# MobleyLab/blues

Measured on AMD Instinct MI355X. Metric: NCMC ns/day (23k-atom toluene box, 1000-step switch, RandomLigandRotationMove), aggregate over independent chains, higher is better.
Workload: dtype f32 pair math / f64 accumulation, f64 alchemical+integrator

## Files before the change

blues_amd/csrc/blues_engine.hip:

```cpp
#include <hip/hip_runtime.h>

#include <algorithm>
#include <array>
#include <cmath>
#include <cstdarg>
#include <cstdio>
#include <cstdlib>
#include <cstring>
#include <map>
#include <memory>
#include <numeric>
#include <string>
#include <vector>

#include "../../include/blues_engine.h"
#include "device_common.h"
#include "kernels_alch.h"
#include "kernels_bonded.h"
#include <chrono>
#include <mutex>
#include <thread>
#include <functional>
#include <atomic>
#include <type_traits>
// ... 234 lines not shown
    bool clusters_packed = false;
    double total_mass = 0;
    DBuf<double> d_x[3], d_v[3], d_xbuild[3], d_mass, d_charge, d_sigma, d_eps;
    DBuf<double> d_x_sort[3], d_stage;
    DBuf<unsigned> d_xfer_out;
    DBuf<int> d_edit_idx; DBuf<double> d_edit_xyz;
    std::vector<struct BluesSnapshot*> snap_pool;
    DBuf<AtomF> d_img_f; DBuf<AtomD> d_img_d;
    DBuf<int> d_sorted_of_orig, d_orig_of_sorted, d_tile_atoms, d_jlist, d_jstage, d_jcount, d_batch_slot, d_ex_start, d_ex_idx, d_islot;
    DBuf<unsigned long long> d_mask_pool;
    DBuf<DevFlags> d_flags; DBuf<DevAccum> d_acc; DBuf<long long> d_stamps;
    DBuf<double> d_fpart, d_epart_nb, d_fJ, d_self_part, d_e_part, d_fent, d_ftot, d_alch_self, d_epart_b, d_cm_part, d_trace, d_scratch;
    DBuf<int> d_orig_of_islot, d_row_of_orig, d_mobile_atoms, d_mobile_index, d_exc_owner, d_exc_is_env;
    DBuf<double> d_noise; unsigned noise_draw_base = 0; int n_noise = 0; bool noise_valid = false;
    DBuf<int> d_alch_orig, d_alch_local, d_exc_start, d_exc_partner; DBuf<double> d_exc_params;
    DBuf<int> d_cl_atoms, d_cl_type, d_cl_nc, d_cl_alch, d_cl_mobile, d_cl_sorted; DBuf<double> d_cl_dist;
    DBuf<ClusterRec> d_recs; std::vector<ClusterRec> h_recs;
    std::vector<GenCluster> gen_h; std::vector<GenAtom> gen_atoms_h; std::vector<GenCons> gen_cons_h;
    std::vector<int> gen_tree;
    DBuf<GenCluster> d_gen; DBuf<GenAtom> d_gen_atoms; DBuf<GenCons> d_gen_cons;
    int n_gen() const { return (int)gen_h.size(); }
    int gen_blocks() const { const int wpb = int_threads / 64; return (n_gen() + wpb - 1) / wpb; }
    DBuf<AlchJRec> d_jrec; DBuf<AlchARec> d_arec;
    DBuf<double> d_mom_part; bool vel_clean = false, pass_valid_for_l = true;
    DBuf<FinRec> d_finrecs; std::vector<int> h_row_of_orig, h_row_start;
    template <typename T> struct PmeBufs { DBuf<T> a_re, a_im, b_re, b_im, eterm, tw_cos[3], tw_sin[3], qf_re, qf_im, phi_f; };
    bool pme = false; int pme_K[3] = {0, 0, 0}, pme_order = 5, disp_corr = 0;
    std::vector<int> pme_frozen;
    DBuf<double> d_qn, d_qn_full, d_frec, d_pme_e; DBuf<int> d_pme_frozen; DBuf<unsigned long long> d_pme_acc;
    PmeBufs<float> pme_f; PmeBufs<double> pme_d;
    bool pme_static_valid = false;
    double e_ewald_const = 0.0, e_disp = 0.0;
    DBuf<int> d_row_atom, d_row_start, d_ent_type, d_ent_term, d_ent_role;
    DBuf<int> d_term_atoms[T_NTYPES]; DBuf<double> d_term_params[T_NTYPES];
    int n_terms[T_NTYPES] = {0, 0, 0, 0, 0, 0}; int n_rows = 0; double restr_k = 0;
    int n_cent = 0; DBuf<int> d_cent_atoms; DBuf<double> d_cent_params;
    Program prog; unsigned prog_draw_base = 0; int prog_trace = -1; bool tracing = false;
    int64_t st_passes = 0, st_launches = 0, st_resorts = 0, st_energy_evals = 0, st_reshapes = 0;
    std::vector<int> h_sorted_of_orig, h_orig_of_sorted;

    ~BluesEngine() {
        for (BluesSnapshot* sn : snap_pool) { if (sn->block) hipFree(sn->block); delete sn; }
        for (hipEvent_t e : {ev0, ev1, evFork, evJ1, evJ2, evA, evB}) if (e) hipEventDestroy(e);
        for (hipStream_t q : {s1, s2}) if (q) hipStreamDestroy(q);
    }
};
// ... 774 lines not shown
            A.q = (float)q; A.hs = (float)hs; A.se = (float)se; A.flags = flags; A.orig = o;
        } else {
            AtomD& A = imd[s];
            A.x = u[0]; A.y = u[1]; A.z = u[2]; A.q = q; A.hs = hs; A.se = se; A.flags = flags; A.orig = o; A.pad = 0;
        }
    }
    try {
        if (h->precision == 0) h->d_img_f.upload(imf); else h->d_img_d.upload(imd);
        h->d_sorted_of_orig.upload(h->h_sorted_of_orig); h->d_orig_of_sorted.upload(h->h_orig_of_sorted);
        { std::vector<int> cs(h->clusters.size() * 4, 0);
          for (size_t c = 0; c < h->clusters.size(); c++) for (int a = 0; a < 4; a++) if (h->clusters[c].atoms[a] >= 0) cs[c * 4 + a] = h->h_sorted_of_orig[h->clusters[c].atoms[a]];
          h->d_cl_sorted.upload(cs);
          for (size_t c = 0; c < h->clusters.size(); c++) for (int a = 0; a < 4; a++) {
              const int at = h->clusters[c].atoms[a];
              h->h_recs[c].sorted[a] = cs[c * 4 + a]; h->h_recs[c].islot[a] = at >= 0 ? islot[at] : -1;
              const int row = at >= 0 && !h->h_row_of_orig.empty() ? h->h_row_of_orig[at] : -1;
              h->h_recs[c].e0[a] = row >= 0 ? h->h_row_start[row] : 0; h->h_recs[c].e1[a] = row >= 0 ? h->h_row_start[row + 1] : 0;
          }
          h->d_recs.upload(h->h_recs); }
        if (h->n_gen()) { for (GenAtom& R : h->gen_atoms_h) { R.sorted = h->h_sorted_of_orig[R.atom]; R.islot = islot[R.atom]; } h->d_gen_atoms.upload(h->gen_atoms_h); }
        h->d_tile_atoms.upload(tile_atoms); h->d_islot.upload(islot);
        h->d_ex_start.upload(ex_start); h->d_ex_idx.upload(ex_idx);
        h->d_jrec.alloc((size_t)jcap);
        { std::vector<AlchARec> ar(h->alch.size());
          for (size_t a2 = 0; a2 < h->alch.size(); a2++) { AlchARec& r = ar[a2]; const int ao = h->alch[a2]; r.ao = ao; r.asrt = h->h_sorted_of_orig[ao]; r.pad = 0; r.sig = h->T->sigma[ao]; r.eps = std::sqrt(h->T->eps[ao]); r.q = h->T->charge[ao];
            r.has_env_excl = 0; for (int p2 : h->T->excl[ao]) if (h->T->alch_local[p2] < 0) r.has_env_excl = 1; }
          h->d_arec.upload(ar); }
        h->lists_alloc = h->k1_mode == 2 ? std::max(1, h->n_itiles) : 0;
        const int nt_alloc = h->k1_mode == 2 ? h->lists_alloc + 1 : nt;
        h->d_jlist.alloc((size_t)nt_alloc * jcap); h->d_jstage.alloc((size_t)nt_alloc * LIST_WAVES * ((((n + LIST_WAVES - 1) / LIST_WAVES) + 63) & ~63)); h->d_jcount.alloc(nt_alloc); h->d_batch_slot.alloc((size_t)nt_alloc * (jcap / 64));
        h->d_mask_pool.alloc((size_t)nt_alloc * MASK_QUOTA * 64);
        h->d_fpart.alloc((size_t)h->npart * 3 * h->n_islots);
        if (h->k1_mode == 2) {
            h->d_alist.alloc((size_t)h->n_islots * h->acap); h->d_acount.alloc(h->n_islots); h->d_aself.alloc(h->n_islots);
            {
                std::vector<int> rows((size_t)h->n_islots * SX_ROW, -1);
                for (int q = 0; q < h->n_islots; q++) {
                    int* r = rows.data() + (size_t)q * SX_ROW;
                    const int sidx = tile_atoms[q];
                    r[28] = 0; r[29] = 0x7fffffff; r[30] = -1;
                    if (sidx < 0) continue;
                    int nrow = 0; r[nrow++] = sidx;
                    for (int e = ex_start[sidx]; e < ex_start[sidx + 1]; e++) if (ex_idx[e] != sidx && nrow < SX_MAX) r[nrow++] = ex_idx[e];
                    r[28] = nrow;
                    for (int e = 0; e < nrow; e++) { r[29] = std::min(r[29], r[e]); r[30] = std::max(r[30], r[e]); }
                }
// ... 188 lines not shown
    h->prog.n = 0; h->prog_trace = -1; h->prog_draw_base = h->h_draw;
    HIP_OK(h, hipGetLastError());
    return 0;
}

static int emit(BluesEngine* h, int op) {
    if (h->prog.n == 0) h->prog_draw_base = h->h_draw;
    if (h->prog.n >= MAX_OPS) { if (flush_program(h)) return 1; h->prog_draw_base = h->h_draw; }
    h->prog.ops[h->prog.n++] = (unsigned char)op;
    if (op == OP_O || op == OP_L) h->h_draw++;
    return 0;
}

static ListArgs make_list_args(BluesEngine* h) {
    ListArgs a; memset(&a, 0, sizeof a);
    a.n = h->n; a.n_tiles = h->n_tiles; a.n_itiles = h->n_itiles; a.jcap = h->jcap; a.pool_cap = h->pool_cap;
    a.tile_atoms = h->d_tile_atoms.p; a.jlist = h->d_jlist.p; a.jstage = h->d_jstage.p; a.jcount = h->d_jcount.p; a.batch_slot = h->d_batch_slot.p;
    a.mask_pool = h->d_mask_pool.p; a.batch_req = batch_req_ptr(h); a.ex_start = h->d_ex_start.p; a.ex_idx = h->d_ex_idx.p; a.flags = h->d_flags.p;
    for (int k = 0; k < 3; k++) { a.x[k] = h->d_x[k].p; a.xbuild[k] = h->d_xbuild[k].p; }
    a.fJ = h->d_fJ.p; a.n_fJ = 9 * h->n;
    a.alch_jrec = h->alch.empty() ? nullptr : (void*)h->d_jrec.p; a.p_sigma = h->d_sigma.p; a.p_eps = h->d_eps.p; a.p_charge = h->d_charge.p;
    if (h->k1_mode == 2) { a.alist = h->d_alist.p; a.acount = h->d_acount.p; a.acap = h->acap; }
    a.S = h->S; a.n_lists = h->n_lists; a.hint_count = h->hint_count; a.no_sphere = h->tune.no_sphere;
    if (h->k1_mode == 2 && h->prune_on) { a.pneed = h->d_pneed.p; a.plist = h->d_plist.p; a.pcount = h->d_pcount.p; for (int k = 0; k < 3; k++) a.xprune[k] = h->d_xprune[k].p; }
    if (h->k1_mode == 2) { a.pimg4 = h->d_pimg4.p; a.pimg2 = h->d_pimg2.p; a.mlist = h->d_mlist.p; a.mcount = h->d_mcount.p; a.mcap = h->mcap; a.aself = h->d_aself.p; a.pimgb = h->d_pimgb.p; a.sx_row = h->d_sx_row.p; a.pf_reach = h->alist_pf_reach; }
    return a;
}

static FragArgs make_frag_args(BluesEngine* h) {
    FragArgs a; memset(&a, 0, sizeof a);
    if (h->k1_mode != 3) return a;
    a.F = h->frag_F; a.NI = h->frag_NI; a.ifrag = h->d_ifrag.p; a.nblk = h->frag_nblk; a.n = h->n; a.ocap = h->frag_ocap; a.icap = h->frag_icap; a.fpw = h->frag_fpw; a.nwg = h->frag_nwg; a.n_islots = h->n_islots;
    a.fimg = h->d_fimg.p; a.ljtab = h->d_ljtab.p; a.ntypes = h->frag_ntypes; a.sp_start = h->d_sp_start.p; a.sp_ent = h->d_sp_ent.p; a.bb = h->d_fbb.p; a.fpos0 = h->d_fpos0.p;
    a.olist = h->d_olist.p; a.ocount = h->d_ocount.p; a.ilist = h->d_ilist.p; a.icount = h->d_icount.p; a.xprune = h->d_xprune_s.p;
    const double ro = h->cutoff + h->skin, ri = h->cutoff + std::min(h->frag_m, h->skin);
    a.ro2 = (float)(ro * ro) * 1.0001f + 1e-5f; a.ri2 = (float)(ri * ri) * 1.0001f + 1e-5f;
    {
        const double rof = h->cutoff + 0.5 * h->skin, rif = h->cutoff + 0.5 * std::min(h->frag_m, h->skin);
        a.ro2_f = (float)(rof * rof) * 1.0001f + 1e-5f; a.ri2_f = (float)(rif * rif) * 1.0001f + 1e-5f;
    }
    a.ptrig2 = h->frag_m < h->skin ? (float)(0.25 * h->frag_m * h->frag_m) : 1e30f;
    for (int k = 0; k < 3; k++) a.scale[k] = (float)(h->box[k] / 4294967296.0);
    a.flags = h->d_flags.p; a.batch_req = batch_req_ptr(h); a.fpart = h->d_fpart.p; a.epart = h->d_epart_nb.p;
    a.half_min_edge = (float)(0.5 * std::min(h->box[0], std::min(h->box[1], h->box[2])));
    a.count_builds = h->n_tiles == 0;
    a.hint_blocks = h->frag_nblk < 64 ? 0x7fffffff : std::max(48, h->frag_nblk * 85 / 100);
// ... 307 lines not shown
        else hipLaunchKernelGGL(k_alchemical<false>, dim3(h->k2_nblocks_env + 1), dim3(256), 0, h->cur, A);
    }
    h->st_launches++;
    HIP_OK(h, hipGetLastError());
    return 0;
}

static AlchArgs make_alch_args(BluesEngine* h, const double ls[3], const double le[3], int slot_mask) {
    AlchArgs A; memset(&A, 0, sizeof A);
    A.jrec = h->d_jrec.p; A.arec = h->d_arec.p;
    A.n = h->n; A.n_alch = (int)h->alch.size(); A.PA = h->PA; A.jcap = h->jcap; A.nblocks_env = h->k2_nblocks_env; A.jiter = h->k2_jiter;
    A.flags_overflow = h->d_flags.p ? &h->d_flags.p->list_overflow : nullptr;
    A.alch_orig = h->d_alch_orig.p; A.jlist = h->d_jlist.p + (size_t)h->n_lists * h->jcap; A.jcount = h->d_jcount.p + h->n_lists;
    A.orig_of_sorted = h->d_orig_of_sorted.p; A.sorted_of_orig = h->d_sorted_of_orig.p;
    for (int k = 0; k < 3; k++) A.x[k] = h->d_x[k].p;
    A.charge = h->d_charge.p; A.sigma = h->d_sigma.p; A.eps = h->d_eps.p; A.ex_start = h->d_ex_start.p; A.ex_idx = h->d_ex_idx.p;
    A.exc_start = h->d_exc_start.p; A.exc_partner = h->d_exc_partner.p; A.exc_owner = h->d_exc_owner.p; A.exc_is_env = h->d_exc_is_env.p; A.exc_params = h->d_exc_params.p;
    A.box = make_box(h); A.rc2 = nocut(h) ? 1e300 : h->cutoff * h->cutoff; A.alpha = h->alpha; A.sc_alpha = h->sc_alpha;
    A.pme = h->nb_method == BLUES_NB_PME_DIRECT; A.annih_elec = h->annih_elec; A.annih_ster = h->annih_ster; A.slot_mask = slot_mask; A.check_env_excl = h->check_env_excl;
    for (int s = 0; s < 3; s++) { A.ls[s] = ls[s]; A.le[s] = le[s]; }
    A.fJ = h->d_fJ.p; A.self_part = h->d_self_part.p; A.e_part = h->d_e_part.p;
    A.img = h->precision == 0 ? h->d_img_f.p : nullptr;
    for (int k = 0; k < 3; k++) A.fscale[k] = (float)(h->box[k] / 4294967296.0);
    return A;
}

static BondedArgs make_bonded_args(BluesEngine* h) {
    BondedArgs B; memset(&B, 0, sizeof B);
    B.n_rows = h->n_rows; B.row_atom = h->d_row_atom.p; B.row_start = h->d_row_start.p;
    B.ent_type = h->d_ent_type.p; B.ent_term = h->d_ent_term.p; B.ent_role = h->d_ent_role.p;
    for (int ty = 0; ty < T_NTYPES; ty++) { B.n_terms[ty] = h->n_terms[ty]; B.atoms[ty] = h->d_term_atoms[ty].p; B.params[ty] = h->d_term_params[ty].p; }
    B.restr_k = h->restr_k; B.ewald_alpha = h->alpha;
    for (int k = 0; k < 3; k++) B.x[k] = h->d_x[k].p;
    B.box = make_box(h); B.periodic = h->nb_method == BLUES_NB_PME_DIRECT; B.fent = h->d_fent.p; B.n_entries = h->n_entries; B.n = h->n; B.epart = h->d_epart_b.p;
    B.n_mobile = (int)h->mobile.size(); B.n_noise = h->n_noise; B.mobile_atoms = h->d_mobile_atoms.p; B.noise = h->d_noise.p;
    B.n_cent = h->n_cent; B.cent_atoms = h->d_cent_atoms.p; B.cent_params = h->d_cent_params.p;
    B.seed = h->seed; B.stream = (unsigned)h->replica * 4u; B.draw_base = h->h_draw; B.n_entry_blocks = (h->n_entries + 127) / 128;
    return B;
}

static int launch_bonded(BluesEngine* h, bool with_noise) {
    BondedArgs B = make_bonded_args(h);
    const int nb_noise = with_noise ? ((int)h->mobile.size() * h->n_noise + 127) / 128 : 0;
    if (with_noise) { h->noise_draw_base = h->h_draw; h->noise_valid = true; }
    if (B.n_entry_blocks + nb_noise > 0) {
        BondedDyn D; D.draw_base = B.draw_base; D.n_entry_blocks = B.n_entry_blocks;
// ... 1876 lines not shown
    else if (k == "nprop") *value = h->nprop;
    else if (k == "prop") *value = h->h_prop;
    else if (k == "prop_lambda_min") *value = h->prop_min;
    else if (k == "prop_lambda_max") *value = h->prop_max;
    else if (k == "Enew" || k == "Eold") {
        double E; if (total_energy(h, &E)) return 1;
        if (read_acc(h, &a)) return 1;
        *value = (k == "Enew") ? E : E - a.dE_last;
    }
    else if (k == "heat") { if (h->led_flags & LED_HEAT) { if (read_acc(h, &a)) return 1; *value = a.heat; } else *value = 0.0; }
    else if (k == "kT") *value = h->kT;
    else if (h->switch_mode != BLUES_SWITCH_NONE && (k == "total_work" || k == "Epert" || k == "initial_energy" || k == "final_energy" || k == "accept" || k == "naccept" || k == "ntrials" || k == "psteps")) {
        if (k == "total_work") { if (read_acc(h, &a)) return 1; *value = a.protocol_work + h->sw_shadow; }
        else if (k == "Epert") *value = h->sw_Epert;
        else if (k == "initial_energy") *value = h->sw_Einit;
        else if (k == "final_energy") { if (h->h_step == 0) *value = 0.0; else if (h->psteps > 0) *value = h->sw_Epert; else if (total_energy(h, value)) return 1; }
        else if (k == "accept") *value = h->sw_accept;
        else if (k == "naccept") *value = h->sw_naccept;
        else if (k == "ntrials") *value = h->sw_ntrials;
        else *value = h->psteps;
    }
    else if (k == "lambda_sterics") *value = h->cur_ls;
    else if (k == "lambda_electrostatics") *value = h->cur_le;
    else E_FAIL(h, "unknown global variable '%s'", name);
    return 0;
}

int blues_set_global(BluesEngine* h, const char* name, double value) {
    HIP_OK(h, hipSetDevice(h->device));
    std::string k(name);
    if (k == "atom_list_prefilter") { h->alist_pf_reach = value <= 0.0 ? -1.0f : (float)(std::min(value, 1e5) * 1e-3); return 0; }
    if (k == "protocol_work" || (k == "shadow_work" && (h->led_flags & LED_SHADOW)) || (k == "heat" && (h->led_flags & LED_HEAT))) {
        DevAccum a; if (read_acc(h, &a)) return 1;
        if (k == "protocol_work") a.protocol_work = value; else if (k == "heat") a.heat = value; else a.shadow_work = value;
        HIP_OK(h, hipMemcpy(h->d_acc.p, &a, sizeof a, hipMemcpyHostToDevice));
        h->acc_cache_valid = false;
    }
    else if (k == "step") h->h_step = (int)value;
    else if (k == "lambda") h->h_lambda = value;
    else if (k == "lambda_step") { h->h_lambda_step = (int)value; parameters_changed(h); }
    else if (k == "first_step") h->h_first_step = (int)value;
    else if (k == "prop") h->h_prop = (int)value;
    else if (k == "nprop") h->nprop = (int)value;
    else if (k == "perturbed_pe") h->h_perturbed = value;
    else if (k == "unperturbed_pe") { h->h_unperturbed = value; }
    else if (k == "shadow_work") { if (h->switch_mode != BLUES_SWITCH_NONE) h->sw_shadow = value; else if (value != 0.0) E_FAIL(h, "shadow work is not measured (measure_shadow_work=False)"); }
    else if (h->switch_mode != BLUES_SWITCH_NONE && (k == "total_work" || k == "naccept" || k == "ntrials")) {
        if (k == "naccept") h->sw_naccept = (int)value; else if (k == "ntrials") h->sw_ntrials = (int)value;
    }
    else if (k == "lambda_sterics") { h->cur_ls = value; parameters_changed(h); }
    else if (k == "lambda_electrostatics") { h->cur_le = value; parameters_changed(h); }
    else E_FAIL(h, "global variable '%s' cannot be set", name);
    return 0;
// ... 730 lines not shown
```

blues_amd/csrc/kernels_alch.h:

```cpp
#pragma once
#include "device_common.h"

#define K2_NE 6
#define K2_STAGE 256
#define K2_NP 9
__host__ __device__ inline int k2_env_blocks(int count, int PA, int jiter) { const int jpb = (256 / PA) * jiter; return (count + jpb - 1) / jpb; }

struct AlchJRec { int jo, jsrt; double sig, eps, q; };
struct AlchARec { int ao, asrt, has_env_excl, pad; double sig, eps, q; };

struct AlchArgs {
    const AlchJRec* jrec; const AlchARec* arec;
    int n, n_alch, PA, jcap, nblocks_env, jiter;
    const int* alch_orig;
    const int* jlist;
    const int* jcount;
    const int* orig_of_sorted;
    const int* sorted_of_orig;
    const double* x[3];
    const double* charge; const double* sigma; const double* eps;
    const int* ex_start; const int* ex_idx;
    const int* exc_start;
    const int* exc_partner;
    const int* exc_owner;
    const int* exc_is_env;
    const double* exc_params;
    Box3 box;
    double rc2, alpha, sc_alpha;
    int pme, annih_elec, annih_ster, slot_mask;
    int check_env_excl;
    double ls[3], le[3];
    double* fJ;
    double* self_part;
    double* e_part;
    int* flags_overflow;
    const AtomF* img;
    float fscale[3];
};

__device__ inline bool excluded_sorted(const int* ex_start, const int* ex_idx, int a_sorted, int j_sorted) {
    bool ex = false;
    for (int e = ex_start[a_sorted]; e < ex_start[a_sorted + 1]; e++) ex |= (ex_idx[e] == j_sorted);
    return ex;
}

template <bool FAST, int MASK = -1, int FORM = 0>
__device__ __forceinline__ bool alchemical_body(AlchArgs& A, const int block_id) {
    auto slot_on = [&](int s) -> bool { return MASK >= 0 ? ((MASK >> s) & 1) != 0 : ((A.slot_mask >> s) & 1) != 0; };
    const int tid = threadIdx.x, lane = tid & 63, wv = tid >> 6;
    const int PA = A.PA;
    const int a = tid & (PA - 1);
    __shared__ double s_self[4][9][64];
    __shared__ double s_e[4][K2_NE];
    __shared__ double s_exc[9][256];
    using FT = typename std::conditional<FAST, float, double>::type;
    FT f[3][3];
#pragma unroll
    for (int s = 0; s < 3; s++) { f[s][0] = f[s][1] = f[s][2] = (FT)0; }
    double e[K2_NE];
#pragma unroll
// ... 481 lines not shown
                }
            }
        }
        __syncthreads();
    }
    if (tid < A.PA) {
#pragma unroll
        for (int q = 0; q < 9; q++) A.self_part[(size_t)q * A.PA + tid] = (tid < A.n_alch && slot_on(q / 3)) ? (double)(long long)S.fa[q][tid] * (1.0 / K2D_FIX) : 0.0;
    }
#pragma unroll
    for (int q = 0; q < K2_NE; q++) e[q] = wave_sum(e[q]);
    if (lane == 0) for (int q = 0; q < K2_NE; q++) S.e[wv][q] = e[q];
    __syncthreads();
    if (tid < K2_NE) { double t = 0.0; for (int w = 0; w < K2D_WAVES; w++) t += S.e[w][tid]; A.e_part[tid] = t; }
    if (tid < 3) { double t = 0.0; for (int a = 0; a < A.n_alch; a++) t += (double)(long long)S.fa[tid][a] * (1.0 / K2D_FIX); A.e_part[K2_NE + tid] = slot_on(0) ? t : 0.0; }
    NB_STAMP(blockIdx.x == 0 && threadIdx.x == 0, 41);
}

#define K2F_THREADS 512
#define K2F_WAVES (K2F_THREADS / 64)
#define K2F_JC 2432
#define K2F_MOB 288
#define K2F_RING 128
#define K2F_FIX 8192.0f
template <int NS> struct K2FLds {
    uint4 r4[K2F_JC];
    float2 r2[K2F_JC];
    unsigned short mslot[K2F_JC];
    int fj[3 * NS][K2F_MOB];
    unsigned short ring[K2F_WAVES][K2F_RING];
    int mcnt[(K2F_JC + 63) / 64 + 2];
    unsigned xa[3][16]; float aq[16], ahs[16], ase[16];
    float fa[16][9];
    double e[K2F_WAVES][4];
};
static_assert(sizeof(K2FLds<2>) <= 76 * 1024, "two workgroups of the fp32 dense alchemical kernel per CU, with room for the allocation granule");

template <int MASK>
__device__ __forceinline__ void alchemical_dense32_body(AlchArgs& A) {
    constexpr int NS = MASK == 5 ? 2 : (MASK == 2 ? 1 : 3);
    auto slot_on = [&](int s) -> bool { return MASK >= 0 ? ((MASK >> s) & 1) != 0 : ((A.slot_mask >> s) & 1) != 0; };
    auto slot_ix = [&](int s) -> int { return MASK == 5 ? (s >> 1) : (MASK == 2 ? 0 : s); };
    extern __shared__ __align__(16) unsigned char k2d_smem[];
    K2FLds<NS>& S = *reinterpret_cast<K2FLds<NS>*>(k2d_smem);
    const int tid = threadIdx.x, lane = tid & 63, wv = tid >> 6;
    const bool stamp_wg = blockIdx.x == (gridDim.x * 5u) / 8u;
    NB_STAMP(stamp_wg && tid == 0, 32);
    const int count = *A.jcount;
    if (count <= 0) return;
    const AtomF* __restrict__ img = A.img;
    const bool no_elec = A.le[0] == 0.0 && A.le[1] == 0.0 && A.le[2] == 0.0, same_ls = A.ls[0] == A.ls[1] && A.ls[1] == A.ls[2];
    const float sA[3] = {(float)(A.sc_alpha * (1.0 - A.ls[0])), (float)(A.sc_alpha * (1.0 - A.ls[1])), (float)(A.sc_alpha * (1.0 - A.ls[2]))};
    const float ls[3] = {(float)A.ls[0], (float)A.ls[1], (float)A.ls[2]}, le[3] = {(float)A.le[0], (float)A.le[1], (float)A.le[2]};
    const float dA01 = (float)(A.sc_alpha * (A.ls[1] - A.ls[0])), dA12 = (float)(A.sc_alpha * (A.ls[2] - A.ls[1]));
    const float dl01 = (float)(A.ls[1] - A.ls[0]), dl12 = (float)(A.ls[2] - A.ls[1]);
    const float rc2 = (float)A.rc2, alpha = (float)A.alpha, c2 = TWO_OVER_SQRT_PI_F * (float)A.alpha;
    const float sc0 = A.fscale[0], sc1 = A.fscale[1], sc2 = A.fscale[2];
    if (tid < 16) {
        const bool on = tid < A.n_alch;
        const AlchARec ar = A.arec[on ? tid : 0];
        const AtomF me = img[ar.asrt];
        S.xa[0][tid] = me.x; S.xa[1][tid] = me.y; S.xa[2][tid] = me.z;
        S.aq[tid] = on ? (float)(ar.q * sqrt(ONE_4PI_EPS0)) : 0.0f; S.ahs[tid] = on ? (float)(0.5 * ar.sig) : 0.0f; S.ase[tid] = on ? (float)(2.0 * ar.eps) : 0.0f;
    }
    for (int w = tid; w < 16 * 9; w += K2F_THREADS) S.fa[w / 9][w % 9] = 0.0f;
    double eC = 0.0, eS0 = 0.0, eD01 = 0.0, eD12 = 0.0;
    constexpr int NIT = (K2F_JC + K2F_THREADS - 1) / K2F_THREADS;
    for (int j0 = 0; j0 < count; j0 += K2F_JC) {
        const int nst = min(K2F_JC, count - j0), nchunk = (nst + 63) >> 6;
        for (int w = tid; w < 3 * NS * K2F_MOB; w += K2F_THREADS) S.fj[w / K2F_MOB][w % K2F_MOB] = 0;
        int js[NIT];
#pragma unroll
        for (int it = 0; it < NIT; it++) { const int k = it * K2F_THREADS + tid; js[it] = k < nst ? A.jlist[j0 + k] : -1; }
        bool mob[NIT]; int mrank[NIT];
#pragma unroll
        for (int it = 0; it < NIT; it++) {
            const int k = it * K2F_THREADS + tid, ch = k >> 6;
            mob[it] = false;
            if (k < K2F_JC) {
                if (js[it] >= 0) {
                    const uint4 lo = *reinterpret_cast<const uint4*>(&img[js[it]]);
                    const uint4 hi = *(reinterpret_cast<const uint4*>(&img[js[it]]) + 1);
                    S.r4[k] = lo; S.r2[k] = make_float2(__uint_as_float(hi.x), __uint_as_float(hi.y));
                    mob[it] = (hi.z & FLAG_MOBILE) != 0;
                }
            }
            const unsigned long long b = __ballot(mob[it]);
            mrank[it] = __popcll(b & ((1ull << lane) - 1ull));
            if (lane == 0 && k < K2F_JC) S.mcnt[ch] = __popcll(b);
        }
        __syncthreads();
        {
            int c = lane < (K2F_JC + 63) / 64 ? S.mcnt[lane] : 0, inc = c;
#pragma unroll
            for (int o = 1; o < 64; o <<= 1) { const int t = __shfl_up(inc, o, 64); if (lane >= o) inc += t; }
            const int exc = inc - c;
#pragma unroll
            for (int it = 0; it < NIT; it++) {
                const int k = it * K2F_THREADS + tid, ch = k >> 6;
                const int ms = __shfl(exc, min(ch, 63), 64) + mrank[it];
                if (k < K2F_JC) S.mslot[k] = (mob[it] && ms < K2F_MOB) ? (unsigned short)ms : (unsigned short)0xffff;
            }
        }
        __syncthreads();
        NB_STAMP(stamp_wg && tid == 0, 33);
        for (int a = wv; a < A.n_alch; a += K2F_WAVES) {
            const unsigned xa = S.xa[0][a], ya = S.xa[1][a], za = S.xa[2][a];
            const float qa = S.aq[a], hsa = S.ahs[a], sea = S.ase[a];
            float fa[NS][3];
#pragma unroll
            for (int s = 0; s < NS; s++) { fa[s][0] = fa[s][1] = fa[s][2] = 0.0f; }
            unsigned short* const ring = S.ring[wv];
            int head = 0, fill = 0;
            auto pairs = [&](int nvalid) {
                const bool valid = lane < nvalid;
                const int k = valid ? (int)ring[(head + lane) & (K2F_RING - 1)] : 0;
                const uint4 p = S.r4[k]; const float2 t = S.r2[k];
                const float dx = (float)(int)(xa - p.x) * sc0, dy = (float)(int)(ya - p.y) * sc1, dz = (float)(int)(za - p.z) * sc2;
                const float r2 = fmaf(dz, dz, fmaf(dy, dy, dx * dx));
                float ft[NS];
#pragma unroll
                for (int s = 0; s < NS; s++) ft[s] = 0.0f;
                if (valid) {
                    const float sig = hsa + t.x, eps4 = sea * t.y, qq = qa * __uint_as_float(p.w);
                    float fc = 0.0f;
                    if (!no_elec && qq != 0.0f) {
                        const float inv_r = __builtin_amdgcn_rsqf(r2), inv_r2 = inv_r * inv_r, arr = alpha * (r2 * inv_r);
                        const float ex = __expf(-arr * arr), ec = erfc_scaled_f(arr) * ex;
                        eC += (double)(qq * ec * inv_r);
                        fc = qq * fmaf(c2, ex, ec * inv_r) * inv_r2;
                    }
                    float fs[3] = {0.0f, 0.0f, 0.0f};
                    if (eps4 != 0.0f) {
                        const float inv_s2 = __builtin_amdgcn_rcpf(fmaxf(sig * sig, 1e-12f)), q2 = r2 * inv_s2, q4 = q2 * q2, q6 = q4 * q2;
                        const float g6 = 6.0f * eps4 * q4 * inv_s2;
                        const float den0 = sA[0] + q6, x0 = __builtin_amdgcn_rcpf(den0);
// ... 8 lines not shown
                            eD01 += (double)(eps4 * fmaf(ls[1] * d01, x0 + x1 - 1.0f, dl01 * u0));
                            eD12 += (double)(eps4 * fmaf(ls[2] * d12, x1 + x2 - 1.0f, dl12 * u1));
                            fs[1] = ls[1] * g6 * fmaf(2.0f, x1, -1.0f) * x1 * x1;
                            fs[2] = ls[2] * g6 * fmaf(2.0f, x2, -1.0f) * x2 * x2;
                        }
                    }
#pragma unroll
                    for (int s = 0; s < 3; s++) if (slot_on(s)) ft[slot_ix(s)] = fmaf(le[s], fc, fs[s]);
                }
                const unsigned ms = valid ? (unsigned)S.mslot[k] : 0xffffu;
#pragma unroll
                for (int s = 0; s < 3; s++) {
                    if (!slot_on(s)) continue;
                    const int q = slot_ix(s);
                    const float fx = ft[q] * dx, fy = ft[q] * dy, fz = ft[q] * dz;
                    fa[q][0] += fx; fa[q][1] += fy; fa[q][2] += fz;
                    if (ms != 0xffffu) {
                        atomicAdd(&S.fj[3 * q + 0][ms], __float2int_rn(-fx * K2F_FIX));
                        atomicAdd(&S.fj[3 * q + 1][ms], __float2int_rn(-fy * K2F_FIX));
                        atomicAdd(&S.fj[3 * q + 2][ms], __float2int_rn(-fz * K2F_FIX));
                    }
                }
            };
            for (int ch = 0; ch < nchunk; ch++) {
                const int k = ch * 64 + lane;
                const uint4 p = S.r4[min(k, nst - 1)];
                const float dx = (float)(int)(xa - p.x) * sc0, dy = (float)(int)(ya - p.y) * sc1, dz = (float)(int)(za - p.z) * sc2;
                const bool hit = k < nst && fmaf(dz, dz, fmaf(dy, dy, dx * dx)) < rc2;
                const unsigned long long b = __ballot(hit);
                if (hit) ring[(head + fill + __popcll(b & ((1ull << lane) - 1ull))) & (K2F_RING - 1)] = (unsigned short)k;
                fill += __popcll(b);
                if (fill >= 64) {
                    __builtin_amdgcn_fence(__ATOMIC_ACQ_REL, "wavefront");
                    pairs(64);
                    head = (head + 64) & (K2F_RING - 1); fill -= 64;
                }
            }
            if (fill > 0) { __builtin_amdgcn_fence(__ATOMIC_ACQ_REL, "wavefront"); pairs(fill); }
#pragma unroll
            for (int s = 0; s < 3; s++) {
                if (!slot_on(s)) continue;
                const int q = slot_ix(s);
#pragma unroll
                for (int c3 = 0; c3 < 3; c3++) { const float v = wave_sum_dpp_f32(fa[q][c3]); if (lane == 0) S.fa[a][s * 3 + c3] += v; }
            }
            NB_STAMP(stamp_wg && lane == 0 && wv == 0, 34 + min(a / K2F_WAVES, 1));
        }
        NB_STAMP(stamp_wg && lane == 0, 36 + min(wv, 7));
        __syncthreads();
#pragma unroll
        for (int it = 0; it < NIT; it++) {
            const int k = it * K2F_THREADS + tid;
            if (k < nst && mob[it]) {
                const unsigned ms = S.mslot[k];
                if (ms == 0xffffu) { if (A.flags_overflow) A.flags_overflow[0] = 1; continue; }
#pragma unroll
                for (int s = 0; s < 3; s++) {
                    if (!slot_on(s)) continue;
#pragma unroll
                    for (int c3 = 0; c3 < 3; c3++) A.fJ[(size_t)(s * 3 + c3) * A.n + js[it]] = (double)S.fj[3 * slot_ix(s) + c3][ms] * (1.0 / (double)K2F_FIX);
                }
            }
        }
        __syncthreads();
    }
    if (tid < A.PA) {
#pragma unroll
        for (int q = 0; q < 9; q++) A.self_part[(size_t)q * A.PA + tid] = (tid < A.n_alch && tid < 16 && slot_on(q / 3)) ? (double)S.fa[tid][q] : 0.0;
    }
    eC = wave_sum(eC); eS0 = wave_sum(eS0); eD01 = wave_sum(eD01); eD12 = wave_sum(eD12);
    if (lane == 0) { S.e[wv][0] = eC; S.e[wv][1] = eS0; S.e[wv][2] = eD01; S.e[wv][3] = eD12; }
    __syncthreads();
    if (tid == 0) {
        double t[4] = {0.0, 0.0, 0.0, 0.0};
        for (int w = 0; w < K2F_WAVES; w++) for (int q = 0; q < 4; q++) t[q] += S.e[w][q];
        A.e_part[0] = t[0]; A.e_part[1] = t[1]; A.e_part[2] = t[1] + t[2]; A.e_part[3] = t[1] + t[2] + t[3];
        A.e_part[4] = 0.0; A.e_part[5] = 0.0;
    }
    if (tid < 3) { double t = 0.0; for (int a = 0; a < A.n_alch && a < 16; a++) t += (double)S.fa[a][tid]; A.e_part[K2_NE + tid] = slot_on(0) ? t : 0.0; }
    NB_STAMP(stamp_wg && tid == 0, 60);
}

template <int MASK>
__global__ void __launch_bounds__(K2F_THREADS, 4) k_alchemical_dense32(AlchArgs A) { alchemical_dense32_body<MASK>(A); }

template <int MASK>
__global__ void __launch_bounds__(K2D_THREADS) k_alchemical_dense(AlchArgs A) { alchemical_dense_body<MASK>(A); }

template <bool FAST, int FORM = 0>
__global__ void __launch_bounds__(256) k_alchemical(AlchArgs A) { alchemical_blocks<FAST, -1, FORM>(A, blockIdx.x, gridDim.x - 1); }
```

blues_amd/csrc/kernels_nb.h:

```cpp
#pragma once
#include "device_common.h"


struct DevFlags {
    unsigned list_gen, req_gen;
    int list_overflow;
    int constraint_fail;
    int nan_flag;
    int resort_hint;
    int builds;
    int prunes;
    int prune_req;
};

struct ListArgs {
    int n, n_tiles, n_itiles, jcap, pool_cap;
    const int* tile_atoms;
    int* jlist;
    int* jstage;
    void* alch_jrec;
    const double* p_sigma; const double* p_eps; const double* p_charge;
    int* jcount;
    int* batch_slot;
    unsigned long long* mask_pool;
    const int* batch_req;
    const int* ex_start;
    const int* ex_idx;
    DevFlags* flags;
    const double* x[3];
    double* xbuild[3];
    double* fJ;
    int n_fJ;
    unsigned short* alist;
    int* acount;
    int acap;
    int no_sphere;
    int hint_count;
    int S, n_lists;
    int* pneed; unsigned short* plist; int* pcount; unsigned* xprune[3];
    uint4* pimg4; float2* pimg2; int* mlist; int* mcount; int mcap;
    unsigned short* aself;
    uint4* pimgb;
    const int* sx_row;
    float pf_reach;
};

#define MASK_QUOTA 24
#define LIST_WAVES 16
#ifndef LIST_PREFETCH
#define LIST_PREFETCH 4
#endif
#define LIST_THREADS (LIST_WAVES * 64)
#define ATOM_LIST_WAVES 4
#define ATOM_LIST_THREADS (ATOM_LIST_WAVES * 64)
#define ATOM_LIST_U 2
#define ATOM_LIST_PARTS (64 / (ATOM_LIST_WAVES * ATOM_LIST_U))
#define ATOM_SLOT(part, wv, u) ((part) * (64 / ATOM_LIST_PARTS) + (wv) * ATOM_LIST_U + (u))
#define ATOM_LIST_RING 128
#define LIST_LDS 8192
#define NB_LQ_BYTES 51200
#define NB_JCAP_MAX 6400
#define NB_LDS_TAIL 512
#define NB_ENT(k) ((unsigned short)((k) << 3))
#define NB_IDX(e) ((int)(e) >> 3)

template <typename R>
// ... 116 lines not shown
            const unsigned long long bal = __ballot(pass);
            if (pass) stage[wcount + __popcll(bal & ((1ull << lane) - 1ull))] = j;
            wcount += __popcll(bal);
        }
    }
    if (lane == 0) s_wcount[wv] = wcount;
    NB_STAMP(t == 0 && tid == 0, 2);
    __syncthreads();
    NB_STAMP(t == 0 && tid == 0, 3);
    {
        int off = 0;
        for (int w = 0; w < wv; w++) off += s_wcount[w];
        for (int k = lane; k < wcount; k += 64) if (off + k < a.jcap) jl[off + k] = stage[k];
        if (tid == 0) { int tot = 0; for (int w = 0; w < LIST_WAVES; w++) tot += s_wcount[w]; s_total = tot; }
    }
    __threadfence_block();
    __syncthreads();
    int count = s_total;
    if (t == 0 && tid == 0) a.flags->builds++;
    const int cap_eff = (!alch_tile && a.alist && a.pimg4) ? a.jcap - 1 : a.jcap;
    if (count > cap_eff) { if (tid == 0) a.flags->list_overflow = 1; count = cap_eff; }
    else if (count > a.hint_count && tid == 0) a.flags->resort_hint = 1;
    if (tid == 0) a.jcount[t] = count;
    const int nb = (count + 63) >> 6;
    const int nbmax = a.jcap >> 6;
    for (int b = tid; b < nbmax; b += LIST_THREADS) { s_need[b] = 0; a.batch_slot[t * nbmax + b] = -1; }
    __syncthreads();
    if (alch_tile) {
        struct JR { int jo, jsrt; double sig, eps, q; };
        JR* jr = (JR*)a.alch_jrec;
        if (jr) for (int k = tid; k < count; k += LIST_THREADS) {
            const int js = jl[k], jo = img[js].orig;
            JR r; r.jo = jo; r.jsrt = js | ((img[js].flags & FLAG_MOBILE) ? 0x40000000 : 0);
            r.sig = a.p_sigma[jo]; r.eps = sqrt(a.p_eps[jo]); r.q = a.p_charge[jo];
            jr[k] = r;
        }
        return;
    }

    NB_STAMP(t == 0 && tid == 0, 4);
    if (a.alist && a.pimg4) {
        if constexpr (sizeof(ufix) == 4) {
            __shared__ int s_mc;
            if (tid == 0) s_mc = 0;
            __syncthreads();
            uint4* g4 = a.pimg4 + (size_t)t * a.jcap; float2* g2 = a.pimg2 + (size_t)t * a.jcap; int* ml = a.mlist + (size_t)t * a.mcap * 2;
// ... 908 lines not shown
```

Measured before the change: 575,700.

## Cache a pruned alchemical neighbor subset, with a Coulomb-only tail, across alchemical kernel steps

The f32 dense alchemical kernel now builds a persistent 'keep' list of environment atoms within cutoff plus the ligand's reach plus a margin. The list is split into LJ-bearing atoms and charge-only atoms, and charge-only atoms take a cheaper Coulomb-only pair path. Later calls reuse the kept list while the ligand stays inside the recorded reach, which skips rescanning and regathering the full neighbor list. A list rebuild invalidates the cache. This adds header bookkeeping, extra global writes on rebuild, and a tunable margin that trades reuse rate against kept-list size.

```diff
diff --git a/blues_amd/csrc/blues_engine.hip b/blues_amd/csrc/blues_engine.hip
--- a/blues_amd/csrc/blues_engine.hip
+++ b/blues_amd/csrc/blues_engine.hip
@@ -280,6 +280,8 @@
     int n_gen() const { return (int)gen_h.size(); }
     int gen_blocks() const { const int wpb = int_threads / 64; return (n_gen() + wpb - 1) / wpb; }
     DBuf<AlchJRec> d_jrec; DBuf<AlchARec> d_arec;
+    DBuf<int> d_k2keep;
+    float k2_keep_margin = 0.10f;
     DBuf<double> d_mom_part; bool vel_clean = false, pass_valid_for_l = true;
     DBuf<FinRec> d_finrecs; std::vector<int> h_row_of_orig, h_row_start;
     template <typename T> struct PmeBufs { DBuf<T> a_re, a_im, b_re, b_im, eterm, tw_cos[3], tw_sin[3], qf_re, qf_im, phi_f; };
@@ -1100,6 +1102,12 @@
         h->d_tile_atoms.upload(tile_atoms); h->d_islot.upload(islot);
         h->d_ex_start.upload(ex_start); h->d_ex_idx.upload(ex_idx);
         h->d_jrec.alloc((size_t)jcap);
+        if (h->k2_f32) {
+            std::vector<int> kh((size_t)K2F_KEEP_HDR + K2F_JC, 0);
+            kh[0] = -1;
+            if (h->d_k2keep.p && hipMemcpy(&kh[5], h->d_k2keep.p + 5, sizeof(int), hipMemcpyDeviceToHost) != hipSuccess) throw std::string("hipMemcpy D2H failed");
+            h->d_k2keep.upload(kh);
+        } else h->d_k2keep.release();
         { std::vector<AlchARec> ar(h->alch.size());
           for (size_t a2 = 0; a2 < h->alch.size(); a2++) { AlchARec& r = ar[a2]; const int ao = h->alch[a2]; r.ao = ao; r.asrt = h->h_sorted_of_orig[ao]; r.pad = 0; r.sig = h->T->sigma[ao]; r.eps = std::sqrt(h->T->eps[ao]); r.q = h->T->charge[ao];
             r.has_env_excl = 0; for (int p2 : h->T->excl[ao]) if (h->T->alch_local[p2] < 0) r.has_env_excl = 1; }
@@ -1334,6 +1342,7 @@
     a.alch_jrec = h->alch.empty() ? nullptr : (void*)h->d_jrec.p; a.p_sigma = h->d_sigma.p; a.p_eps = h->d_eps.p; a.p_charge = h->d_charge.p;
     if (h->k1_mode == 2) { a.alist = h->d_alist.p; a.acount = h->d_acount.p; a.acap = h->acap; }
     a.S = h->S; a.n_lists = h->n_lists; a.hint_count = h->hint_count; a.no_sphere = h->tune.no_sphere;
+    a.alch_keep = h->d_k2keep.p;
     if (h->k1_mode == 2 && h->prune_on) { a.pneed = h->d_pneed.p; a.plist = h->d_plist.p; a.pcount = h->d_pcount.p; for (int k = 0; k < 3; k++) a.xprune[k] = h->d_xprune[k].p; }
     if (h->k1_mode == 2) { a.pimg4 = h->d_pimg4.p; a.pimg2 = h->d_pimg2.p; a.mlist = h->d_mlist.p; a.mcount = h->d_mcount.p; a.mcap = h->mcap; a.aself = h->d_aself.p; a.pimgb = h->d_pimgb.p; a.sx_row = h->d_sx_row.p; a.pf_reach = h->alist_pf_reach; }
     return a;
@@ -1687,6 +1696,7 @@
     A.fJ = h->d_fJ.p; A.self_part = h->d_self_part.p; A.e_part = h->d_e_part.p;
     A.img = h->precision == 0 ? h->d_img_f.p : nullptr;
     for (int k = 0; k < 3; k++) A.fscale[k] = (float)(h->box[k] / 4294967296.0);
+    A.keep = h->k2_f32 ? h->d_k2keep.p : nullptr; A.keep_margin = h->k2_keep_margin;
     return A;
 }
 
@@ -3609,6 +3619,11 @@
     }
     else if (k == "lambda_sterics") *value = h->cur_ls;
     else if (k == "lambda_electrostatics") *value = h->cur_le;
+    else if (k == "alch_keep_derivations") {
+        int v = 0;
+        if (h->d_k2keep.p) { if (flush_program(h)) return 1; HIP_OK(h, hipStreamSynchronize(h->stream)); HIP_OK(h, hipMemcpy(&v, h->d_k2keep.p + 5, sizeof v, hipMemcpyDeviceToHost)); }
+        *value = v;
+    }
     else E_FAIL(h, "unknown global variable '%s'", name);
     return 0;
 }
@@ -3616,6 +3631,7 @@
 int blues_set_global(BluesEngine* h, const char* name, double value) {
     HIP_OK(h, hipSetDevice(h->device));
     std::string k(name);
+    if (k == "alch_keep_margin") { h->k2_keep_margin = value <= 0.0 ? 0.0f : (float)(std::min(value, 1e4) * 1e-3); h->args_epoch++; return 0; }
     if (k == "atom_list_prefilter") { h->alist_pf_reach = value <= 0.0 ? -1.0f : (float)(std::min(value, 1e5) * 1e-3); return 0; }
     if (k == "protocol_work" || (k == "shadow_work" && (h->led_flags & LED_SHADOW)) || (k == "heat" && (h->led_flags & LED_HEAT))) {
         DevAccum a; if (read_acc(h, &a)) return 1;
diff --git a/blues_amd/csrc/kernels_alch.h b/blues_amd/csrc/kernels_alch.h
--- a/blues_amd/csrc/kernels_alch.h
+++ b/blues_amd/csrc/kernels_alch.h
@@ -36,6 +36,8 @@
     int* flags_overflow;
     const AtomF* img;
     float fscale[3];
+    int* keep;
+    float keep_margin;
 };
 
 __device__ inline bool excluded_sorted(const int* ex_start, const int* ex_idx, int a_sorted, int j_sorted) {
@@ -563,6 +565,8 @@
 #define K2F_JC 2432
 #define K2F_MOB 288
 #define K2F_RING 128
+#define K2F_KEEP_HDR 8
+#define K2F_KEEP_GUARD 1e-4f
 #define K2F_FIX 8192.0f
 template <int NS> struct K2FLds {
     uint4 r4[K2F_JC];
@@ -590,6 +594,13 @@
     const int count = *A.jcount;
     if (count <= 0) return;
     const AtomF* __restrict__ img = A.img;
+    int* const keep = A.keep;
+    const bool use_keep = keep && count <= 2 * K2F_JC;
+    int kh[7] = {-1, 0, 0, 0, 0, 0, 0};
+    if (use_keep) {
+#pragma unroll
+        for (int q = 0; q < 7; q++) if (q != 5) kh[q] = keep[q];
+    }
     const bool no_elec = A.le[0] == 0.0 && A.le[1] == 0.0 && A.le[2] == 0.0, same_ls = A.ls[0] == A.ls[1] && A.ls[1] == A.ls[2];
     const float sA[3] = {(float)(A.sc_alpha * (1.0 - A.ls[0])), (float)(A.sc_alpha * (1.0 - A.ls[1])), (float)(A.sc_alpha * (1.0 - A.ls[2]))};
     const float ls[3] = {(float)A.ls[0], (float)A.ls[1], (float)A.ls[2]}, le[3] = {(float)A.le[0], (float)A.le[1], (float)A.le[2]};
@@ -605,26 +616,104 @@
         S.aq[tid] = on ? (float)(ar.q * sqrt(ONE_4PI_EPS0)) : 0.0f; S.ahs[tid] = on ? (float)(0.5 * ar.sig) : 0.0f; S.ase[tid] = on ? (float)(2.0 * ar.eps) : 0.0f;
     }
     for (int w = tid; w < 16 * 9; w += K2F_THREADS) S.fa[w / 9][w % 9] = 0.0f;
-    double eC = 0.0, eS0 = 0.0, eD01 = 0.0, eD12 = 0.0;
+    double eC = 0.0, eCc = 0.0, eS0 = 0.0, eD01 = 0.0, eD12 = 0.0;
     constexpr int NIT = (K2F_JC + K2F_THREADS - 1) / K2F_THREADS;
-    for (int j0 = 0; j0 < count; j0 += K2F_JC) {
-        const int nst = min(K2F_JC, count - j0), nchunk = (nst + 63) >> 6;
+    const int* src = A.jlist; int total = count;
+    int keptL = -1, keptC = 0;
+    bool staged = false;
+    if (use_keep) {
+        __syncthreads();
+        const int al = min(lane, 15); const bool aon = lane < A.n_alch && lane < 16;
+        const unsigned ax = S.xa[0][al], ay = S.xa[1][al], az = S.xa[2][al];
+        auto reach_of = [&](unsigned cx, unsigned cy, unsigned cz) -> float {
+            const float dx = (float)(int)(ax - cx) * sc0, dy = (float)(int)(ay - cy) * sc1, dz = (float)(int)(az - cz) * sc2;
+            float d2 = aon ? fmaf(dz, dz, fmaf(dy, dy, dx * dx)) : 0.0f;
+#pragma unroll
+            for (int o = 1; o < 16; o <<= 1) d2 = fmaxf(d2, __shfl_xor(d2, o, 64));
+            return sqrtf(__shfl(d2, 0, 64));
+        };
+        const int kc = __builtin_amdgcn_readfirstlane(kh[0]);
+        const unsigned hx = (unsigned)kh[1], hy = (unsigned)kh[2], hz = (unsigned)kh[3];
+        const float hreach = __int_as_float(kh[4]);
+        const float far = reach_of(hx, hy, hz);
+        const bool valid = __builtin_amdgcn_readfirstlane((int)(kc >= 0 && kc <= K2F_JC && A.keep_margin > 0.0f && far <= hreach)) != 0;
+        if (valid) { src = keep + K2F_KEEP_HDR; keptL = kc; keptC = __builtin_amdgcn_readfirstlane(kh[6]); keptC = max(0, min(keptC, K2F_JC - keptL)); total = 1; }
+        else if (kc != -2) {
+            unsigned c0[3];
+            {
+                const unsigned x0[3] = {S.xa[0][0], S.xa[1][0], S.xa[2][0]}, xm[3] = {ax, ay, az};
+#pragma unroll
+                for (int c3 = 0; c3 < 3; c3++) {
+                    int lo = aon ? (int)(xm[c3] - x0[c3]) : 0, hi = lo;
+#pragma unroll
+                    for (int o = 1; o < 16; o <<= 1) { lo = min(lo, __shfl_xor(lo, o, 64)); hi = max(hi, __shfl_xor(hi, o, 64)); }
+                    c0[c3] = (unsigned)__shfl((int)(x0[c3] + (unsigned)lo + (((unsigned)hi - (unsigned)lo) >> 1)), 0, 64);
+                }
+            }
+            const float R0 = reach_of(c0[0], c0[1], c0[2]), m = fmaxf(A.keep_margin, 0.0f);
+            const float thr = sqrtf(rc2) + R0 + m + K2F_KEEP_GUARD, thr2 = thr * thr;
+            int runL = 0, runC = 0;
+            int jn = tid < count ? A.jlist[tid] : -1, jnn = K2F_THREADS + tid < count ? A.jlist[K2F_THREADS + tid] : -1;
+            uint4 lon = make_uint4(0u, 0u, 0u, 0u), hin = lon;
+            if (jn >= 0) { lon = *reinterpret_cast<const uint4*>(&img[jn]); hin = *(reinterpret_cast<const uint4*>(&img[jn]) + 1); }
+            for (int base = 0, par = 0; base < count; base += K2F_THREADS, par ^= 1) {
+                const int j = jn; const uint4 lo = lon, hi = hin;
+                jn = jnn;
+                { const int i2 = base + 2 * K2F_THREADS + tid; jnn = i2 < count ? A.jlist[i2] : -1; }
+                if (jn >= 0) { lon = *reinterpret_cast<const uint4*>(&img[jn]); hin = *(reinterpret_cast<const uint4*>(&img[jn]) + 1); }
+                const bool mobj = j >= 0 && (hi.z & FLAG_MOBILE) != 0;
+                bool kp = false;
+                if (j >= 0) {
+                    const float dx = (float)(int)(lo.x - c0[0]) * sc0, dy = (float)(int)(lo.y - c0[1]) * sc1, dz = (float)(int)(lo.z - c0[2]) * sc2;
+                    kp = mobj || fmaf(dz, dz, fmaf(dy, dy, dx * dx)) < thr2;
+                }
+                const bool ljj = hi.y != 0u;
+                const unsigned long long b = __ballot(kp), bl = __ballot(kp && ljj), below = (1ull << lane) - 1ull;
+                if (lane == 0) { S.mcnt[(par * 2 + 0) * K2F_WAVES + wv] = __popcll(bl); S.mcnt[(par * 2 + 1) * K2F_WAVES + wv] = __popcll(b & ~bl); }
+                __syncthreads();
+                int offL = runL, offC = runC, totL = 0, totC = 0;
+#pragma unroll
+                for (int w = 0; w < K2F_WAVES; w++) {
+                    const int cl = S.mcnt[(par * 2 + 0) * K2F_WAVES + w], cc = S.mcnt[(par * 2 + 1) * K2F_WAVES + w];
+                    offL += w < wv ? cl : 0; offC += w < wv ? cc : 0; totL += cl; totC += cc;
+                }
+                const int pos = ljj ? offL + __popcll(bl & below) : K2F_JC - 1 - (offC + __popcll(b & ~bl & below));
+                if (kp && pos >= 0 && pos < K2F_JC) {
+                    S.r4[pos] = lo; S.r2[pos] = make_float2(__uint_as_float(hi.x), __uint_as_float(hi.y));
+                    S.mslot[pos] = mobj ? (unsigned short)1 : (unsigned short)0;
+                    keep[K2F_KEEP_HDR + pos] = j;
+                }
+                runL += __builtin_amdgcn_readfirstlane(totL); runC += __builtin_amdgcn_readfirstlane(totC);
+            }
+            __syncthreads();
+            const bool fits = runL + runC <= K2F_JC;
+            if (tid == 0) {
+                keep[1] = (int)c0[0]; keep[2] = (int)c0[1]; keep[3] = (int)c0[2];
+                keep[4] = __float_as_int(R0 + m - K2F_KEEP_GUARD); keep[5] = keep[5] + 1;
+                keep[6] = runC;
+                keep[0] = fits ? runL : -2;
+            }
+            if (fits) { staged = true; src = keep + K2F_KEEP_HDR; keptL = runL; keptC = runC; total = 1; }
+        }
+    }
+    for (int j0 = 0; j0 < total; j0 += K2F_JC) {
+        const int nL = keptL >= 0 ? keptL : min(K2F_JC, total - j0), nC = keptL >= 0 ? keptC : 0;
         for (int w = tid; w < 3 * NS * K2F_MOB; w += K2F_THREADS) S.fj[w / K2F_MOB][w % K2F_MOB] = 0;
         int js[NIT];
 #pragma unroll
-        for (int it = 0; it < NIT; it++) { const int k = it * K2F_THREADS + tid; js[it] = k < nst ? A.jlist[j0 + k] : -1; }
+        for (int it = 0; it < NIT; it++) { const int k = it * K2F_THREADS + tid; js[it] = (k < nL || (k >= K2F_JC - nC && k < K2F_JC)) ? src[j0 + k] : -1; }
         bool mob[NIT]; int mrank[NIT];
 #pragma unroll
         for (int it = 0; it < NIT; it++) {
             const int k = it * K2F_THREADS + tid, ch = k >> 6;
             mob[it] = false;
             if (k < K2F_JC) {
-                if (js[it] >= 0) {
+                if (js[it] >= 0 && !staged) {
                     const uint4 lo = *reinterpret_cast<const uint4*>(&img[js[it]]);
                     const uint4 hi = *(reinterpret_cast<const uint4*>(&img[js[it]]) + 1);
                     S.r4[k] = lo; S.r2[k] = make_float2(__uint_as_float(hi.x), __uint_as_float(hi.y));
                     mob[it] = (hi.z & FLAG_MOBILE) != 0;
-                }
+                } else if (js[it] >= 0) mob[it] = S.mslot[k] != 0;
             }
             const unsigned long long b = __ballot(mob[it]);
             mrank[it] = __popcll(b & ((1ull << lane) - 1ull));
@@ -653,6 +742,7 @@
             for (int s = 0; s < NS; s++) { fa[s][0] = fa[s][1] = fa[s][2] = 0.0f; }
             unsigned short* const ring = S.ring[wv];
             int head = 0, fill = 0;
+            float fcs[3] = {0.0f, 0.0f, 0.0f};
             auto pairs = [&](int nvalid) {
                 const bool valid = lane < nvalid;
                 const int k = valid ? (int)ring[(head + lane) & (K2F_RING - 1)] : 0;
@@ -707,11 +797,39 @@
                     }
                 }
             };
-            for (int ch = 0; ch < nchunk; ch++) {
+            auto pairs_coul = [&](int nvalid) {
+                const bool valid = lane < nvalid;
+                const int k = valid ? (int)ring[(head + lane) & (K2F_RING - 1)] : 0;
+                const uint4 p = S.r4[k];
+                const float dx = (float)(int)(xa - p.x) * sc0, dy = (float)(int)(ya - p.y) * sc1, dz = (float)(int)(za - p.z) * sc2;
+                const float r2 = fmaf(dz, dz, fmaf(dy, dy, dx * dx));
+                const float qq = qa * __uint_as_float(p.w);
+                float fc = 0.0f;
+                if (valid && qq != 0.0f) {
+                    const float inv_r = __builtin_amdgcn_rsqf(r2), inv_r2 = inv_r * inv_r, arr = alpha * (r2 * inv_r);
+                    const float ex = __expf(-arr * arr), ec = erfc_scaled_f(arr) * ex;
+                    eCc += (double)(qq * ec * inv_r);
+                    fc = qq * fmaf(c2, ex, ec * inv_r) * inv_r2;
+                }
+                fcs[0] = fmaf(fc, dx, fcs[0]); fcs[1] = fmaf(fc, dy, fcs[1]); fcs[2] = fmaf(fc, dz, fcs[2]);
+                const unsigned ms = valid ? (unsigned)S.mslot[k] : 0xffffu;
+                if (ms != 0xffffu) {
+#pragma unroll
+                    for (int s = 0; s < 3; s++) {
+                        if (!slot_on(s)) continue;
+                        const int q = slot_ix(s);
+                        const float g = le[s] * fc;
+                        atomicAdd(&S.fj[3 * q + 0][ms], __float2int_rn(-(g * dx) * K2F_FIX));
+                        atomicAdd(&S.fj[3 * q + 1][ms], __float2int_rn(-(g * dy) * K2F_FIX));
+                        atomicAdd(&S.fj[3 * q + 2][ms], __float2int_rn(-(g * dz) * K2F_FIX));
+                    }
+                }
+            };
+            for (int ch = 0; ch < ((nL + 63) >> 6); ch++) {
                 const int k = ch * 64 + lane;
-                const uint4 p = S.r4[min(k, nst - 1)];
+                const uint4 p = S.r4[min(k, nL - 1)];
                 const float dx = (float)(int)(xa - p.x) * sc0, dy = (float)(int)(ya - p.y) * sc1, dz = (float)(int)(za - p.z) * sc2;
-                const bool hit = k < nst && fmaf(dz, dz, fmaf(dy, dy, dx * dx)) < rc2;
+                const bool hit = k < nL && fmaf(dz, dz, fmaf(dy, dy, dx * dx)) < rc2;
                 const unsigned long long b = __ballot(hit);
                 if (hit) ring[(head + fill + __popcll(b & ((1ull << lane) - 1ull))) & (K2F_RING - 1)] = (unsigned short)k;
                 fill += __popcll(b);
@@ -722,12 +840,30 @@
                 }
             }
             if (fill > 0) { __builtin_amdgcn_fence(__ATOMIC_ACQ_REL, "wavefront"); pairs(fill); }
+            if (!no_elec && nC > 0) {
+                head = 0; fill = 0;
+                for (int ch = 0; ch < ((nC + 63) >> 6); ch++) {
+                    const int i = ch * 64 + lane, k = K2F_JC - 1 - min(i, nC - 1);
+                    const uint4 p = S.r4[k];
+                    const float dx = (float)(int)(xa - p.x) * sc0, dy = (float)(int)(ya - p.y) * sc1, dz = (float)(int)(za - p.z) * sc2;
+                    const bool hit = i < nC && fmaf(dz, dz, fmaf(dy, dy, dx * dx)) < rc2;
+                    const unsigned long long b = __ballot(hit);
+                    if (hit) ring[(head + fill + __popcll(b & ((1ull << lane) - 1ull))) & (K2F_RING - 1)] = (unsigned short)k;
+                    fill += __popcll(b);
+                    if (fill >= 64) {
+                        __builtin_amdgcn_fence(__ATOMIC_ACQ_REL, "wavefront");
+                        pairs_coul(64);
+                        head = (head + 64) & (K2F_RING - 1); fill -= 64;
+                    }
+                }
+                if (fill > 0) { __builtin_amdgcn_fence(__ATOMIC_ACQ_REL, "wavefront"); pairs_coul(fill); }
+            }
 #pragma unroll
             for (int s = 0; s < 3; s++) {
                 if (!slot_on(s)) continue;
                 const int q = slot_ix(s);
 #pragma unroll
-                for (int c3 = 0; c3 < 3; c3++) { const float v = wave_sum_dpp_f32(fa[q][c3]); if (lane == 0) S.fa[a][s * 3 + c3] += v; }
+                for (int c3 = 0; c3 < 3; c3++) { const float v = wave_sum_dpp_f32(fmaf(le[s], fcs[c3], fa[q][c3])); if (lane == 0) S.fa[a][s * 3 + c3] += v; }
             }
             NB_STAMP(stamp_wg && lane == 0 && wv == 0, 34 + min(a / K2F_WAVES, 1));
         }
@@ -736,7 +872,7 @@
 #pragma unroll
         for (int it = 0; it < NIT; it++) {
             const int k = it * K2F_THREADS + tid;
-            if (k < nst && mob[it]) {
+            if (mob[it]) {
                 const unsigned ms = S.mslot[k];
                 if (ms == 0xffffu) { if (A.flags_overflow) A.flags_overflow[0] = 1; continue; }
 #pragma unroll
@@ -753,7 +889,7 @@
 #pragma unroll
         for (int q = 0; q < 9; q++) A.self_part[(size_t)q * A.PA + tid] = (tid < A.n_alch && tid < 16 && slot_on(q / 3)) ? (double)S.fa[tid][q] : 0.0;
     }
-    eC = wave_sum(eC); eS0 = wave_sum(eS0); eD01 = wave_sum(eD01); eD12 = wave_sum(eD12);
+    eC = wave_sum(eC + eCc); eS0 = wave_sum(eS0); eD01 = wave_sum(eD01); eD12 = wave_sum(eD12);
     if (lane == 0) { S.e[wv][0] = eC; S.e[wv][1] = eS0; S.e[wv][2] = eD01; S.e[wv][3] = eD12; }
     __syncthreads();
     if (tid == 0) {
diff --git a/blues_amd/csrc/kernels_nb.h b/blues_amd/csrc/kernels_nb.h
--- a/blues_amd/csrc/kernels_nb.h
+++ b/blues_amd/csrc/kernels_nb.h
@@ -42,6 +42,7 @@
     unsigned short* aself;
     uint4* pimgb;
     const int* sx_row;
+    int* alch_keep;
     float pf_reach;
 };
 
@@ -204,6 +205,7 @@
     if (count > cap_eff) { if (tid == 0) a.flags->list_overflow = 1; count = cap_eff; }
     else if (count > a.hint_count && tid == 0) a.flags->resort_hint = 1;
     if (tid == 0) a.jcount[t] = count;
+    if (alch_tile && tid == 0 && a.alch_keep) a.alch_keep[0] = -1;
     const int nb = (count + 63) >> 6;
     const int nbmax = a.jcap >> 6;
     for (int b = tid; b < nbmax; b += LIST_THREADS) { s_need[b] = 0; a.batch_slot[t * nbmax + b] = -1; }
```

After: 582,300 (median of 6 runs). 1.01x the previous value.
